# krzkro4122/vit-gan

Hardware: AMD Instinct MI355X
Metric: images/sec (G+D step) ViTGAN 32x32 patch4 dim384 (higher is better)
Workload: dtype bf16; 1 GPU; C2: CIFAR-10-shaped 3x32x32, patch 4 (65 tokens), E=384, 4 heads, 6 blocks ViT discriminator + SLN/SIREN generator (z=1024, 32 tokens, 4 blocks), full alternating G+D step, AdamW; fp8_attention=False, per_gpu_batch=256, global_batch=256, loss=ns, parallelism=dp1, hip_graph=True, compress_mapping_grad=False, fused_real_fake_pass=True, losses_finite=True

## Files before the change

vit-gan_amd/csrc/attention.hip:

```cpp
#include "vg_attn.h"
#include "vg_kernels.h"

typedef long fp8x8;
__device__ __forceinline__ fp8x8 to_fp8(float a0, float a1, float a2, float a3, float a4, float a5, float a6, float a7) {
  int lo = 0, hi = 0;
  lo = __builtin_amdgcn_cvt_pk_fp8_f32(a0, a1, lo, false);
  lo = __builtin_amdgcn_cvt_pk_fp8_f32(a2, a3, lo, true);
  hi = __builtin_amdgcn_cvt_pk_fp8_f32(a4, a5, hi, false);
  hi = __builtin_amdgcn_cvt_pk_fp8_f32(a6, a7, hi, true);
  return (fp8x8)(((unsigned long)(unsigned)hi << 32) | (unsigned long)(unsigned)lo);
}
__device__ __forceinline__ fp8x8 to_fp8(bf16x8 v) {
  return to_fp8(vg_bf2f(v[0]), vg_bf2f(v[1]), vg_bf2f(v[2]), vg_bf2f(v[3]), vg_bf2f(v[4]), vg_bf2f(v[5]), vg_bf2f(v[6]), vg_bf2f(v[7]));
}
__device__ __forceinline__ fp8x8 pack_pair_fp8(f32x4 a, f32x4 b, float mul) {
  return to_fp8(a[0] * mul, a[1] * mul, a[2] * mul, a[3] * mul, b[0] * mul, b[1] * mul, b[2] * mul, b[3] * mul);
}
__device__ __forceinline__ f32x4 vg_mfma_fp8(fp8x8 a, fp8x8 b, f32x4 c) { return __builtin_amdgcn_mfma_f32_16x16x32_fp8_fp8(a, b, c, 0, 0, 0); }
template <bool FP8>
__device__ __forceinline__ f32x4 score_mfma(bf16x8 a, bf16x8 b, f32x4 c) {
  if constexpr (FP8) return vg_mfma_fp8(to_fp8(a), to_fp8(b), c);
  else return vg_mfma(a, b, c);
}
#define VG_P_FP8_SCALE 256.0f

template <int HE>
__device__ __forceinline__ void row_sqnorms(const unsigned char* img, float* out, int rows, int tid, int nthreads) {
  for (int r = tid; r < rows; r += nthreads) {
    float a = 0.f;
#pragma unroll
    for (int c = 0; c < HE / 8; ++c) {
      const bf16x8 v = *(const bf16x8*)(img + lds_off<HE>(r, 8 * c));
#pragma unroll
      for (int j = 0; j < 8; ++j) { const float f = vg_bf2f(v[j]); a += f * f; }
    }
    out[r] = a;
  }
}
__device__ __forceinline__ float l2_dist(float qk, float qn, float kn) { return sqrtf(fmaxf(qn + kn - 2.f * qk, 0.f)); }

template <int HE, int NT, bool L2, bool FP8>
__global__ __launch_bounds__(64 * NT) void vg_attn_fwd_kernel(const bf16* __restrict__ qkv, bf16* __restrict__ o,
                                                              float* __restrict__ lse, int B, int S, int H, float scale,
                                                              const void* __restrict__ zeros) {
  constexpr int KS = HE / 32, DT = HE / 16, KP = (NT + 1) / 2, RP = KP * 32, RK = 16 * NT;
  __shared__ __attribute__((aligned(16))) unsigned char sm[(RK + RP) * HE * 2 + (L2 ? RK * 4 : 0)];
  unsigned char* kl = sm;
  unsigned char* vl = sm + RK * HE * 2;
  float* kn = (float*)(sm + (RK + RP) * HE * 2);
  int b, h;
  if (!attn_block(B, H, b, h)) return;
  const int tid = threadIdx.x, lane = tid & 63, qt = tid >> 6;
  const int g = lane >> 4, li = lane & 15;
  const int E = H * HE;
  const size_t ld = 3 * (size_t)E;
  const bf16* qb = qkv + (size_t)b * S * ld + h * HE;
  const bf16* kb = qb + E;
  const bf16* vb = qb + 2 * E;

  bf16x8 qf[KS];
#pragma unroll
  for (int ks = 0; ks < KS; ++ks) qf[ks] = gfrag(qb, ld, 16 * qt, ks, S, lane);
  dma_head<HE, NT>(kl, kb, ld, S, RK, zeros, qt, lane);
  dma_head<HE, NT>(vl, vb, ld, S, RP, zeros, (qt + 2) % NT, lane);
  asm volatile("s_waitcnt vmcnt(0)" ::: "memory");
  __syncthreads();
  float qn = 0.f;
  if (L2) {
    row_sqnorms<HE>(kl, kn, RK, tid, 64 * NT);
#pragma unroll
    for (int ks = 0; ks < KS; ++ks)
#pragma unroll
      for (int j = 0; j < 8; ++j) { const float f = vg_bf2f(qf[ks][j]); qn += f * f; }
    qn = group_sum(qn);
    __syncthreads();
  }

  f32x4 sc[NT];
#pragma unroll
  for (int kt = 0; kt < NT; ++kt) {
    f32x4 a = {0.f, 0.f, 0.f, 0.f};
#pragma unroll
    for (int ks = 0; ks < KS; ++ks) a = score_mfma<FP8>(lfrag_row<HE>(kl, 16 * kt, ks, lane), qf[ks], a);
    sc[kt] = a;
  }
  const int q = 16 * qt + li;
  float m = -INFINITY;
#pragma unroll
  for (int kt = 0; kt < NT; ++kt)
#pragma unroll
    for (int r = 0; r < 4; ++r) {
      const int key = 16 * kt + 4 * g + r;
      const float raw = L2 ? l2_dist(sc[kt][r], qn, kn[key]) : sc[kt][r];
      const float sv = (key < S) ? raw * scale : -INFINITY;
      sc[kt][r] = sv;
      m = fmaxf(m, sv);
    }
  m = group_max(m);
  float l = 0.f;
#pragma unroll
  for (int kt = 0; kt < NT; ++kt)
#pragma unroll
    for (int r = 0; r < 4; ++r) {
      const float p = __expf(sc[kt][r] - m);
      sc[kt][r] = p;
      l += p;
    }
  l = group_sum(l);
  const float inv_l = 1.0f / l;
  if (g == 0 && q < S) lse[((size_t)b * H + h) * S + q] = m + __logf(l);

  f32x4 oa[DT];
#pragma unroll
  for (int dt = 0; dt < DT; ++dt) oa[dt] = (f32x4){0.f, 0.f, 0.f, 0.f};
#pragma unroll
  for (int u = 0; u < KP; ++u) {
    const f32x4 zero = {0.f, 0.f, 0.f, 0.f};
    const f32x4 hi = (2 * u + 1 < NT) ? sc[(2 * u + 1 < NT) ? 2 * u + 1 : 0] : zero;
    if constexpr (FP8) {
      const fp8x8 pf = pack_pair_fp8(sc[2 * u], hi, VG_P_FP8_SCALE);
#pragma unroll
      for (int dt = 0; dt < DT; ++dt) oa[dt] = vg_mfma_fp8(to_fp8(lfrag_tr<HE>(vl, u, 16 * dt, lane)), pf, oa[dt]);
    } else {
      const bf16x8 pf = pack_pair(sc[2 * u], hi);
#pragma unroll
      for (int dt = 0; dt < DT; ++dt) oa[dt] = vg_mfma(lfrag_tr<HE>(vl, u, 16 * dt, lane), pf, oa[dt]);
    }
  }
  store_tiles<DT>(o + ((size_t)b * S + (q < S ? q : 0)) * E + h * HE, oa, FP8 ? inv_l * (1.0f / VG_P_FP8_SCALE) : inv_l, g, q < S);
}

template <int HE, int NT, bool L2, bool FP8>
__global__ __launch_bounds__(64 * NT, 2) void vg_attn_bwd_kernel(const bf16* __restrict__ qkv, const bf16* __restrict__ o,
                                                         const bf16* __restrict__ d_o, const float* __restrict__ lse,
                                                         bf16* __restrict__ dqkv, int B, int S, int H, float scale,
                                                         const void* __restrict__ zeros) {
  constexpr int KS = HE / 32, DT = HE / 16, KP = (NT + 1) / 2, RP = KP * 32;
  constexpr int IMG = RP * HE * 2;
  __shared__ __attribute__((aligned(16))) unsigned char sm[4 * IMG + (L2 ? 4 : 2) * RP * 4];
  unsigned char* lk = sm;
  unsigned char* lv = sm + IMG;
  unsigned char* lq = sm + 2 * IMG;
  unsigned char* ldo = sm + 3 * IMG;
  float* dl = (float*)(sm + 4 * IMG);
  float* ll = dl + RP;
  float* qn_l = ll + RP;
  float* kn_l = qn_l + RP;
  int b, h;
  if (!attn_block(B, H, b, h)) return;
  const int tid = threadIdx.x, lane = tid & 63, wv = tid >> 6;
  const int g = lane >> 4, li = lane & 15;
  const int E = H * HE;
  const size_t ld = 3 * (size_t)E;
  const bf16* qb = qkv + (size_t)b * S * ld + h * HE;
  const bf16* kb = qb + E;
  const bf16* vb = qb + 2 * E;
  const bf16* ob = o + (size_t)b * S * E + h * HE;
  const bf16* dob = d_o + (size_t)b * S * E + h * HE;
  const float* lb = lse + ((size_t)b * H + h) * S;
  bf16* dqb = dqkv + (size_t)b * S * ld + h * HE;
  const f32x4 zero = {0.f, 0.f, 0.f, 0.f};

  bf16x8 of[KS];
#pragma unroll
  for (int ks = 0; ks < KS; ++ks) of[ks] = gfrag(ob, (size_t)E, 16 * wv, ks, S, lane);
  dma_head<HE, NT>(lk, kb, ld, S, RP, zeros, wv, lane);
  dma_head<HE, NT>(lv, vb, ld, S, RP, zeros, (wv + 1) % NT, lane);
  dma_head<HE, NT>(lq, qb, ld, S, RP, zeros, (wv + 2) % NT, lane);
  dma_head<HE, NT>(ldo, dob, (size_t)E, S, RP, zeros, (wv + 3) % NT, lane);
  for (int i = tid; i < RP; i += 64 * NT) ll[i] = (i < S) ? lb[i] : 0.f;
  asm volatile("s_waitcnt vmcnt(0)" ::: "memory");
  __syncthreads();

  bf16x8 qf[KS], dof[KS];
  {
    float dpart = 0.f;
#pragma unroll
    for (int ks = 0; ks < KS; ++ks) {
      qf[ks] = lfrag_row<HE>(lq, 16 * wv, ks, lane);
      dof[ks] = lfrag_row<HE>(ldo, 16 * wv, ks, lane);
#pragma unroll
      for (int j = 0; j < 8; ++j) dpart += vg_bf2f(dof[ks][j]) * vg_bf2f(of[ks][j]);
    }
    const float delta = group_sum(dpart);
    if (g == 0) dl[16 * wv + li] = delta;
  }
  if (L2) { row_sqnorms<HE>(lq, qn_l, RP, tid, 64 * NT); row_sqnorms<HE>(lk, kn_l, RP, tid, 64 * NT); }
  __syncthreads();

  {
    const int qt = wv;
    const int q = 16 * qt + li;
    const float delta = dl[q];
    const float lse_q = ll[q];
    const float qn = L2 ? qn_l[q] : 0.f;
    float wsum = 0.f;
    f32x4 ds[NT];
#pragma unroll
    for (int kt = 0; kt < NT; ++kt) {
      f32x4 st = zero, dpt = zero;
#pragma unroll
      for (int ks = 0; ks < KS; ++ks) {
        st = score_mfma<FP8>(lfrag_row<HE>(lk, 16 * kt, ks, lane), qf[ks], st);
        dpt = vg_mfma(lfrag_row<HE>(lv, 16 * kt, ks, lane), dof[ks], dpt);
      }
      f32x4 kn4 = zero;
      if (L2) kn4 = *(const f32x4*)(kn_l + 16 * kt + 4 * g);
#pragma unroll
      for (int r = 0; r < 4; ++r) {
        const int key = 16 * kt + 4 * g + r;
        const float raw = L2 ? l2_dist(st[r], qn, kn4[r]) : st[r];
        const float p = (key < S && q < S) ? __expf(raw * scale - lse_q) : 0.f;
        float dsv = p * (dpt[r] - delta) * scale;
        if (L2) { dsv = raw > 0.f ? dsv / raw : 0.f; wsum += dsv; }
        ds[kt][r] = dsv;
      }
    }
    if (L2) wsum = group_sum(wsum);
    f32x4 dq[DT];
#pragma unroll
    for (int dt = 0; dt < DT; ++dt) dq[dt] = zero;
#pragma unroll
    for (int u = 0; u < KP; ++u) {
      const bf16x8 dsf = pack_pair(ds[2 * u], (2 * u + 1 < NT) ? ds[(2 * u + 1 < NT) ? 2 * u + 1 : 0] : zero);
#pragma unroll
      for (int dt = 0; dt < DT; ++dt) dq[dt] = vg_mfma(lfrag_tr<HE>(lk, u, 16 * dt, lane), dsf, dq[dt]);
    }
    if (L2) {
#pragma unroll
      for (int dt = 0; dt < DT; ++dt) {
        const bf16x4 qv = *(const bf16x4*)(lq + lds_off<HE>(q, 16 * dt + 4 * g));
#pragma unroll
        for (int r = 0; r < 4; ++r) dq[dt][r] = wsum * vg_bf2f(qv[r]) - dq[dt][r];
      }
    }
    store_tiles<DT>(dqb + (size_t)(q < S ? q : 0) * ld, dq, 1.0f, g, q < S);
  }
  {
    const int kt = wv;
    const int key = 16 * kt + li;
    bf16x8 kf[KS], vf[KS];
#pragma unroll
    for (int ks = 0; ks < KS; ++ks) {
      kf[ks] = lfrag_row<HE>(lk, 16 * kt, ks, lane);
      vf[ks] = lfrag_row<HE>(lv, 16 * kt, ks, lane);
    }
    f32x4 pr[NT], ds[NT];
    const float kn = L2 ? kn_l[key] : 0.f;
    float wsum = 0.f;
#pragma unroll
    for (int qt = 0; qt < NT; ++qt) {
      f32x4 s = zero, dp = zero;
#pragma unroll
      for (int ks = 0; ks < KS; ++ks) {
        s = score_mfma<FP8>(lfrag_row<HE>(lq, 16 * qt, ks, lane), kf[ks], s);
        dp = vg_mfma(lfrag_row<HE>(ldo, 16 * qt, ks, lane), vf[ks], dp);
      }
      const f32x4 lq4 = *(const f32x4*)(ll + 16 * qt + 4 * g);
      const f32x4 dl4 = *(const f32x4*)(dl + 16 * qt + 4 * g);
      f32x4 qn4 = zero;
      if (L2) qn4 = *(const f32x4*)(qn_l + 16 * qt + 4 * g);
#pragma unroll
      for (int r = 0; r < 4; ++r) {
        const int q = 16 * qt + 4 * g + r;
        const bool ok = (q < S) && (key < S);
        const float raw = L2 ? l2_dist(s[r], qn4[r], kn) : s[r];
        const float p = ok ? __expf(raw * scale - lq4[r]) : 0.f;
        pr[qt][r] = p;
        float dsv = p * (dp[r] - dl4[r]) * scale;
        if (L2) { dsv = raw > 0.f ? dsv / raw : 0.f; wsum += dsv; }
        ds[qt][r] = dsv;
      }
    }
    if (L2) wsum = group_sum(wsum);
    f32x4 dv[DT], dk[DT];
#pragma unroll
    for (int dt = 0; dt < DT; ++dt) { dv[dt] = zero; dk[dt] = zero; }
#pragma unroll
    for (int u = 0; u < KP; ++u) {
      const int hi = (2 * u + 1 < NT) ? 2 * u + 1 : 0;
      const bf16x8 pf = pack_pair(pr[2 * u], (2 * u + 1 < NT) ? pr[hi] : zero);
      const bf16x8 dsf = pack_pair(ds[2 * u], (2 * u + 1 < NT) ? ds[hi] : zero);
#pragma unroll
      for (int dt = 0; dt < DT; ++dt) {
        dv[dt] = vg_mfma(lfrag_tr<HE>(ldo, u, 16 * dt, lane), pf, dv[dt]);
        dk[dt] = vg_mfma(lfrag_tr<HE>(lq, u, 16 * dt, lane), dsf, dk[dt]);
      }
    }
    if (L2) {
#pragma unroll
      for (int dt = 0; dt < DT; ++dt) {
        const bf16x4 kv = *(const bf16x4*)(lk + lds_off<HE>(key, 16 * dt + 4 * g));
#pragma unroll
        for (int r = 0; r < 4; ++r) dk[dt][r] = wsum * vg_bf2f(kv[r]) - dk[dt][r];
      }
    }
    bf16* rowp = dqb + (size_t)(key < S ? key : 0) * ld;
    store_tiles<DT>(rowp + E, dk, 1.0f, g, key < S);
    store_tiles<DT>(rowp + 2 * E, dv, 1.0f, g, key < S);
  }
}

#ifndef VG_ATTN_BWD2_WPE
#define VG_ATTN_BWD2_WPE 5
#endif
template <int HE, int NT, bool FP8>
__global__ __launch_bounds__(64 * NT, VG_ATTN_BWD2_WPE) void vg_attn_bwd2_kernel(const bf16* __restrict__ qkv, const bf16* __restrict__ o,
                                                                  const bf16* __restrict__ d_o, const float* __restrict__ lse,
                                                                  bf16* __restrict__ dqkv, int B, int S, int H, float scale,
                                                                  const void* __restrict__ zeros) {
  constexpr int KS = HE / 32, DT = HE / 16, KP = (NT + 1) / 2, RP = KP * 32;
  constexpr int IMG = RP * HE * 2;
  __shared__ __attribute__((aligned(16))) unsigned char sm[2 * IMG + 2 * RP * 4];
  unsigned char* s0 = sm;
  unsigned char* s1 = sm + IMG;
  float* dl = (float*)(sm + 2 * IMG);
  float* ll = dl + RP;
  int b, h;
  if (!attn_block(B, H, b, h)) return;
  const int tid = threadIdx.x, lane = tid & 63, wv = tid >> 6;
  const int g = lane >> 4, li = lane & 15;
  const int E = H * HE;
  const size_t ld = 3 * (size_t)E;
  const bf16* qb = qkv + (size_t)b * S * ld + h * HE;
  const bf16* kb = qb + E;
  const bf16* vb = qb + 2 * E;
  const bf16* ob = o + (size_t)b * S * E + h * HE;
  const bf16* dob = d_o + (size_t)b * S * E + h * HE;
  const float* lb = lse + ((size_t)b * H + h) * S;
  bf16* dqb = dqkv + (size_t)b * S * ld + h * HE;
  const f32x4 zero = {0.f, 0.f, 0.f, 0.f};

  dma_head<HE, NT>(s0, kb, ld, S, RP, zeros, wv, lane);
  dma_head<HE, NT>(s1, vb, ld, S, RP, zeros, (wv + 1) % NT, lane);
  bf16x8 qf[KS], dof[KS];
  {
    bf16x8 of[KS];
#pragma unroll
    for (int ks = 0; ks < KS; ++ks) {
      of[ks] = gfrag(ob, (size_t)E, 16 * wv, ks, S, lane);
      dof[ks] = gfrag(dob, (size_t)E, 16 * wv, ks, S, lane);
      qf[ks] = gfrag(qb, ld, 16 * wv, ks, S, lane);
    }
    for (int i = tid; i < RP; i += 64 * NT) ll[i] = (i < S) ? lb[i] : 0.f;
    float dpart = 0.f;
#pragma unroll
    for (int ks = 0; ks < KS; ++ks) {
#pragma unroll
      for (int j = 0; j < 8; ++j) dpart += vg_bf2f(dof[ks][j]) * vg_bf2f(of[ks][j]);
    }
    const float delta = group_sum(dpart);
    if (g == 0) dl[16 * wv + li] = delta;
  }
  asm volatile("s_waitcnt vmcnt(0)" ::: "memory");
  __syncthreads();

  {
    const int q = 16 * wv + li;
    const float delta = dl[q];
    const float lse_q = ll[q];
    f32x4 ds[NT];
#pragma unroll
    for (int kt = 0; kt < NT; ++kt) {
      f32x4 st = zero, dpt = zero;
#pragma unroll
      for (int ks = 0; ks < KS; ++ks) {
        st = score_mfma<FP8>(lfrag_row<HE>(s0, 16 * kt, ks, lane), qf[ks], st);
        dpt = vg_mfma(lfrag_row<HE>(s1, 16 * kt, ks, lane), dof[ks], dpt);
      }
#pragma unroll
      for (int r = 0; r < 4; ++r) {
        const int key = 16 * kt + 4 * g + r;
        const float p = (key < S && q < S) ? __expf(st[r] * scale - lse_q) : 0.f;
        ds[kt][r] = p * (dpt[r] - delta) * scale;
      }
    }
    bf16x8 dsf[KP];
#pragma unroll
    for (int u = 0; u < KP; ++u) dsf[u] = pack_pair(ds[2 * u], (2 * u + 1 < NT) ? ds[(2 * u + 1 < NT) ? 2 * u + 1 : 0] : zero);
    bf16* rowq = dqb + (size_t)(q < S ? q : 0) * ld;
#pragma unroll
    for (int pp = 0; pp < DT / 2; ++pp) {
      f32x4 dq[2] = {zero, zero};
#pragma unroll
      for (int u = 0; u < KP; ++u) {
        dq[0] = vg_mfma(lfrag_tr<HE>(s0, u, 32 * pp, lane), dsf[u], dq[0]);
        dq[1] = vg_mfma(lfrag_tr<HE>(s0, u, 32 * pp + 16, lane), dsf[u], dq[1]);
      }
      store_tiles<2>(rowq + 32 * pp, dq, 1.0f, g, q < S);
    }
  }
  bf16x8 kf[KS], vf[KS];
#pragma unroll
  for (int ks = 0; ks < KS; ++ks) {
    kf[ks] = lfrag_row<HE>(s0, 16 * wv, ks, lane);
    vf[ks] = lfrag_row<HE>(s1, 16 * wv, ks, lane);
  }
  __syncthreads();
  dma_head<HE, NT>(s0, qb, ld, S, RP, zeros, wv, lane);
  dma_head<HE, NT>(s1, dob, (size_t)E, S, RP, zeros, (wv + 1) % NT, lane);
  asm volatile("s_waitcnt vmcnt(0)" ::: "memory");
  __syncthreads();
  {
    const int key = 16 * wv + li;
    f32x4 pr[NT], ds[NT];
#pragma unroll
    for (int qt = 0; qt < NT; ++qt) {
      f32x4 s = zero, dp = zero;
#pragma unroll
      for (int ks = 0; ks < KS; ++ks) {
        s = score_mfma<FP8>(lfrag_row<HE>(s0, 16 * qt, ks, lane), kf[ks], s);
        dp = vg_mfma(lfrag_row<HE>(s1, 16 * qt, ks, lane), vf[ks], dp);
      }
      const f32x4 lq4 = *(const f32x4*)(ll + 16 * qt + 4 * g);
      const f32x4 dl4 = *(const f32x4*)(dl + 16 * qt + 4 * g);
#pragma unroll
      for (int r = 0; r < 4; ++r) {
        const int q = 16 * qt + 4 * g + r;
        const float p = ((q < S) && (key < S)) ? __expf(s[r] * scale - lq4[r]) : 0.f;
        pr[qt][r] = p;
        ds[qt][r] = p * (dp[r] - dl4[r]) * scale;
      }
    }
    bf16x8 pf[KP], dsf[KP];
#pragma unroll
    for (int u = 0; u < KP; ++u) {
      const int hi = (2 * u + 1 < NT) ? 2 * u + 1 : 0;
      pf[u] = pack_pair(pr[2 * u], (2 * u + 1 < NT) ? pr[hi] : zero);
      dsf[u] = pack_pair(ds[2 * u], (2 * u + 1 < NT) ? ds[hi] : zero);
    }
    bf16* rowp = dqb + (size_t)(key < S ? key : 0) * ld;
#pragma unroll
    for (int pp = 0; pp < DT / 2; ++pp) {
      f32x4 dv[2] = {zero, zero}, dk[2] = {zero, zero};
#pragma unroll
      for (int u = 0; u < KP; ++u) {
#pragma unroll
        for (int t = 0; t < 2; ++t) {
          dv[t] = vg_mfma(lfrag_tr<HE>(s1, u, 32 * pp + 16 * t, lane), pf[u], dv[t]);
          dk[t] = vg_mfma(lfrag_tr<HE>(s0, u, 32 * pp + 16 * t, lane), dsf[u], dk[t]);
        }
      }
      store_tiles<2>(rowp + E + 32 * pp, dk, 1.0f, g, key < S);
      store_tiles<2>(rowp + 2 * E + 32 * pp, dv, 1.0f, g, key < S);
    }
  }
}

template <int HE>
__global__ __launch_bounds__(320, 2) void vg_attn_bwd_bwd2_kernel(const bf16* __restrict__ qkv, const bf16* __restrict__ d_o,
                                                                  const float* __restrict__ lse, const bf16* __restrict__ uqkv,
                                                                  bf16* __restrict__ d_do, bf16* __restrict__ d_qkv, int B, int S, int H,
                                                                  float scale, const void* __restrict__ zeros) {
  constexpr int NT = 5, KS = HE / 32, DT = HE / 16, KP = 3, RP = 96;
  constexpr int IMG = RP * HE * 2;
  __shared__ __attribute__((aligned(16))) unsigned char sm[4 * IMG + 4 * RP * 4];
  unsigned char* i0 = sm;
  unsigned char* i1 = sm + IMG;
  unsigned char* i2 = sm + 2 * IMG;
  unsigned char* i3 = sm + 3 * IMG;
  float* dl = (float*)(sm + 4 * IMG);
  float* gm = dl + RP;
  float* pl = gm + RP;
  float* ll = pl + RP;
  int b, h;
  if (!attn_block(B, H, b, h)) return;
  const int tid = threadIdx.x, lane = tid & 63, wv = tid >> 6;
  const int g = lane >> 4, li = lane & 15;
  const int E = H * HE;
  const size_t ld = 3 * (size_t)E;
  const bf16* qb = qkv + (size_t)b * S * ld + h * HE;
  const bf16* kb = qb + E;
  const bf16* vb = qb + 2 * E;
  const bf16* uqb = uqkv + (size_t)b * S * ld + h * HE;
  const bf16* ukb = uqb + E;
  const bf16* uvb = uqb + 2 * E;
  const bf16* dob = d_o + (size_t)b * S * E + h * HE;
  const float* lb = lse + ((size_t)b * H + h) * S;
  bf16* ddob = d_do + (size_t)b * S * E + h * HE;
  bf16* dqb = d_qkv + (size_t)b * S * ld + h * HE;
  const f32x4 zero = {0.f, 0.f, 0.f, 0.f};

  dma_head<HE, NT>(i0, kb, ld, S, RP, zeros, wv, lane);
  dma_head<HE, NT>(i1, vb, ld, S, RP, zeros, (wv + 1) % NT, lane);
  dma_head<HE, NT>(i2, ukb, ld, S, RP, zeros, (wv + 2) % NT, lane);
  dma_head<HE, NT>(i3, uvb, ld, S, RP, zeros, (wv + 3) % NT, lane);
  bf16x8 qf[KS], dof[KS], uqf[KS];
#pragma unroll
  for (int ks = 0; ks < KS; ++ks) {
    qf[ks] = gfrag(qb, ld, 16 * wv, ks, S, lane);
    dof[ks] = gfrag(dob, (size_t)E, 16 * wv, ks, S, lane);
    uqf[ks] = gfrag(uqb, ld, 16 * wv, ks, S, lane);
  }
  for (int i = tid; i < RP; i += 64 * NT) ll[i] = (i < S) ? lb[i] : 0.f;
  asm volatile("s_waitcnt vmcnt(0)" ::: "memory");
  __syncthreads();

  {
    const int q = 16 * wv + li;
    const float lse_q = ll[q];
    f32x4 Pm[NT], Dm[NT], Gm[NT], Tm[NT];
    float delta = 0.f, gam = 0.f;
#pragma unroll
    for (int kt = 0; kt < NT; ++kt) {
      f32x4 st = zero, dpt = zero, gt = zero, tt = zero;
#pragma unroll
      for (int ks = 0; ks < KS; ++ks) {
        const bf16x8 kr = lfrag_row<HE>(i0, 16 * kt, ks, lane);
        st = vg_mfma(kr, qf[ks], st);
        gt = vg_mfma(kr, uqf[ks], gt);
        gt = vg_mfma(lfrag_row<HE>(i2, 16 * kt, ks, lane), qf[ks], gt);
        dpt = vg_mfma(lfrag_row<HE>(i1, 16 * kt, ks, lane), dof[ks], dpt);
        tt = vg_mfma(lfrag_row<HE>(i3, 16 * kt, ks, lane), dof[ks], tt);
      }
#pragma unroll
      for (int r = 0; r < 4; ++r) {
        const int key = 16 * kt + 4 * g + r;
        const float p = (key < S && q < S) ? __expf(st[r] * scale - lse_q) : 0.f;
        const float gv = gt[r] * scale;
        Pm[kt][r] = p; Dm[kt][r] = dpt[r]; Gm[kt][r] = gv; Tm[kt][r] = tt[r];
        delta += p * dpt[r];
        gam += p * gv;
      }
    }
    delta = group_sum(delta);
    gam = group_sum(gam);
    float pis = 0.f;
#pragma unroll
    for (int kt = 0; kt < NT; ++kt)
#pragma unroll
      for (int r = 0; r < 4; ++r) {
        const float a = Dm[kt][r] - delta;
        const float pie = Tm[kt][r] + Gm[kt][r] * a - gam * Dm[kt][r];
        Tm[kt][r] = pie;
        Dm[kt][r] = a;
        pis += Pm[kt][r] * pie;
      }
    pis = group_sum(pis);
    if (g == 0) { dl[q] = delta; gm[q] = gam; pl[q] = pis; }
#pragma unroll
    for (int kt = 0; kt < NT; ++kt)
#pragma unroll
      for (int r = 0; r < 4; ++r) {
        const float p = Pm[kt][r];
        Gm[kt][r] = p * (Gm[kt][r] - gam);
        Dm[kt][r] = p * Dm[kt][r];
        Tm[kt][r] = p * (Tm[kt][r] - pis);
      }
    bf16x8 pf[KP], hf[KP], dsf[KP], sgf[KP];
#pragma unroll
    for (int u = 0; u < KP; ++u) {
      const bool two = 2 * u + 1 < NT;
      const int hi = two ? 2 * u + 1 : 0;
      pf[u] = pack_pair(Pm[2 * u], two ? Pm[hi] : zero);
      hf[u] = pack_pair(Gm[2 * u], two ? Gm[hi] : zero);
      dsf[u] = pack_pair(Dm[2 * u], two ? Dm[hi] : zero);
      sgf[u] = pack_pair(Tm[2 * u], two ? Tm[hi] : zero);
    }
    bf16* rowo = ddob + (size_t)(q < S ? q : 0) * E;
    bf16* rowq = dqb + (size_t)(q < S ? q : 0) * ld;
#pragma unroll
    for (int pp = 0; pp < DT / 2; ++pp) {
      f32x4 o1[2] = {zero, zero}, o2[2] = {zero, zero};
#pragma unroll
      for (int u = 0; u < KP; ++u)
#pragma unroll
        for (int t = 0; t < 2; ++t) {
          const int d0 = 32 * pp + 16 * t;
          o1[t] = vg_mfma(lfrag_tr<HE>(i3, u, d0, lane), pf[u], o1[t]);
          o1[t] = vg_mfma(lfrag_tr<HE>(i1, u, d0, lane), hf[u], o1[t]);
          o2[t] = vg_mfma(lfrag_tr<HE>(i2, u, d0, lane), dsf[u], o2[t]);
          o2[t] = vg_mfma(lfrag_tr<HE>(i0, u, d0, lane), sgf[u], o2[t]);
        }
      store_tiles<2>(rowo + 32 * pp, o1, 1.0f, g, q < S);
      store_tiles<2>(rowq + 32 * pp, o2, scale, g, q < S);
    }
  }
  bf16x8 kf[KS], vf[KS], ukf[KS], uvf[KS];
#pragma unroll
  for (int ks = 0; ks < KS; ++ks) {
    kf[ks] = lfrag_row<HE>(i0, 16 * wv, ks, lane);
    vf[ks] = lfrag_row<HE>(i1, 16 * wv, ks, lane);
    ukf[ks] = lfrag_row<HE>(i2, 16 * wv, ks, lane);
    uvf[ks] = lfrag_row<HE>(i3, 16 * wv, ks, lane);
  }
  __syncthreads();
  dma_head<HE, NT>(i0, qb, ld, S, RP, zeros, wv, lane);
  dma_head<HE, NT>(i1, dob, (size_t)E, S, RP, zeros, (wv + 1) % NT, lane);
  dma_head<HE, NT>(i2, uqb, ld, S, RP, zeros, (wv + 2) % NT, lane);
  asm volatile("s_waitcnt vmcnt(0)" ::: "memory");
  __syncthreads();
  {
    const int key = 16 * wv + li;
    f32x4 Hm[NT], Dm[NT], Sm[NT];
#pragma unroll
    for (int qt = 0; qt < NT; ++qt) {
      f32x4 st = zero, dpt = zero, gt = zero, tt = zero;
#pragma unroll
      for (int ks = 0; ks < KS; ++ks) {
        const bf16x8 qr = lfrag_row<HE>(i0, 16 * qt, ks, lane);
        const bf16x8 dr = lfrag_row<HE>(i1, 16 * qt, ks, lane);
        st = vg_mfma(qr, kf[ks], st);
        gt = vg_mfma(qr, ukf[ks], gt);
        gt = vg_mfma(lfrag_row<HE>(i2, 16 * qt, ks, lane), kf[ks], gt);
        dpt = vg_mfma(dr, vf[ks], dpt);
        tt = vg_mfma(dr, uvf[ks], tt);
      }
      const f32x4 lq4 = *(const f32x4*)(ll + 16 * qt + 4 * g);
      const f32x4 dl4 = *(const f32x4*)(dl + 16 * qt + 4 * g);
      const f32x4 gm4 = *(const f32x4*)(gm + 16 * qt + 4 * g);
      const f32x4 pl4 = *(const f32x4*)(pl + 16 * qt + 4 * g);
#pragma unroll
      for (int r = 0; r < 4; ++r) {
        const int q = 16 * qt + 4 * g + r;
        const float p = ((q < S) && (key < S)) ? __expf(st[r] * scale - lq4[r]) : 0.f;
        const float gv = gt[r] * scale, a = dpt[r] - dl4[r];
        const float pie = tt[r] + gv * a - gm4[r] * dpt[r];
        Hm[qt][r] = p * (gv - gm4[r]);
        Dm[qt][r] = p * a;
        Sm[qt][r] = p * (pie - pl4[r]);
      }
    }
    bf16x8 hf[KP], dsf[KP], sgf[KP];
#pragma unroll
    for (int u = 0; u < KP; ++u) {
      const bool two = 2 * u + 1 < NT;
      const int hi = two ? 2 * u + 1 : 0;
      hf[u] = pack_pair(Hm[2 * u], two ? Hm[hi] : zero);
      dsf[u] = pack_pair(Dm[2 * u], two ? Dm[hi] : zero);
      sgf[u] = pack_pair(Sm[2 * u], two ? Sm[hi] : zero);
    }
    bf16* rowp = dqb + (size_t)(key < S ? key : 0) * ld;
#pragma unroll
    for (int pp = 0; pp < DT / 2; ++pp) {
      f32x4 dk[2] = {zero, zero}, dv[2] = {zero, zero};
#pragma unroll
      for (int u = 0; u < KP; ++u)
#pragma unroll
        for (int t = 0; t < 2; ++t) {
          const int d0 = 32 * pp + 16 * t;
          dk[t] = vg_mfma(lfrag_tr<HE>(i2, u, d0, lane), dsf[u], dk[t]);
          dk[t] = vg_mfma(lfrag_tr<HE>(i0, u, d0, lane), sgf[u], dk[t]);
          dv[t] = vg_mfma(lfrag_tr<HE>(i1, u, d0, lane), hf[u], dv[t]);
        }
      store_tiles<2>(rowp + E + 32 * pp, dk, scale, g, key < S);
      store_tiles<2>(rowp + 2 * E + 32 * pp, dv, 1.0f, g, key < S);
    }
  }
}

__device__ __attribute__((aligned(16))) unsigned int vg_attn_zero_page[4] = {0u, 0u, 0u, 0u};
static const void* attn_zeros() {
  static void* zp = nullptr;
  if (!zp && hipGetSymbolAddress(&zp, HIP_SYMBOL(vg_attn_zero_page)) != hipSuccess) zp = nullptr;
  return zp;
}

template <int HE, int NT, int MODE>
static int launch_fwd(const bf16* qkv, bf16* o, float* lse, int B, int H, int S, float scale, hipStream_t st) {
  const void* z = attn_zeros();
  if (!z) return -5;
  hipLaunchKernelGGL((vg_attn_fwd_kernel<HE, NT, MODE == 1, MODE == 2>), dim3(attn_grid(B, H)), dim3(64 * NT), 0, st, qkv, o, lse, B, S, H, scale, z);
  return (int)hipGetLastError();
}
template <int HE, int NT, int MODE>
static int launch_bwd(const bf16* qkv, const bf16* o, const bf16* d_o, const float* lse, bf16* dqkv, int B, int H,
                      int S, float scale, hipStream_t st) {
  const void* z = attn_zeros();
  if (!z) return -5;
#ifndef VG_ATTN_BWD_4IMG
  if constexpr (MODE != 1 && NT == 5) {
    hipLaunchKernelGGL((vg_attn_bwd2_kernel<HE, NT, MODE == 2>), dim3(attn_grid(B, H)), dim3(64 * NT), 0, st, qkv, o, d_o, lse, dqkv, B, S, H, scale, z);
    return (int)hipGetLastError();
  }
#endif
  hipLaunchKernelGGL((vg_attn_bwd_kernel<HE, NT, MODE == 1, MODE == 2>), dim3(attn_grid(B, H)), dim3(64 * NT), 0, st, qkv, o, d_o, lse, dqkv, B, S, H, scale, z);
  return (int)hipGetLastError();
}

#define VG_ATTN_BY_NT(FN, HE_, MODE_, ...) return small ? FN<HE_, 2, MODE_>(__VA_ARGS__) : FN<HE_, 5, MODE_>(__VA_ARGS__)
#define VG_ATTN_BY_MODE(FN, HE_, ...)                                  \
  do {                                                                 \
    if (mode == 0) { VG_ATTN_BY_NT(FN, HE_, 0, __VA_ARGS__); }         \
    if (mode == 1) { VG_ATTN_BY_NT(FN, HE_, 1, __VA_ARGS__); }         \
    VG_ATTN_BY_NT(FN, HE_, 2, __VA_ARGS__);                            \
  } while (0)
#define VG_ATTN_DISPATCH(FN, ...)                                      \
  do {                                                                 \
    if (S < 1 || S > 80 || B < 1 || H < 1) return -2;                  \
    if (mode < 0 || mode > 2) return -4;                               \
    const bool small = (S <= 32);                                      \
    if (HE == 96) VG_ATTN_BY_MODE(FN, 96, __VA_ARGS__);                \
    if (HE == 64) VG_ATTN_BY_MODE(FN, 64, __VA_ARGS__);                \
    if (HE == 32) VG_ATTN_BY_MODE(FN, 32, __VA_ARGS__);                \
    return -3;                                                         \
  } while (0)
int vg_attn_fwd_launch(const bf16* qkv, bf16* o, float* lse, int B, int H, int S, int HE, float scale, int mode, hipStream_t st) {
  if (mode == 0 && S > VG_SHORT_MAX_S && S <= VG_ATTN_LONG_MAX_S) return vg_attn_long_fwd_launch(qkv, o, lse, B, H, S, HE, scale, st);
  VG_ATTN_DISPATCH(launch_fwd, qkv, o, lse, B, H, S, scale, st);
}
int vg_attn_bwd_launch(const bf16* qkv, const bf16* o, const bf16* d_o, const float* lse, bf16* dqkv, int B, int H,
                       int S, int HE, float scale, int mode, hipStream_t st) {
  if (mode == 0 && S > VG_SHORT_MAX_S && S <= VG_ATTN_LONG_MAX_S) return vg_attn_long_bwd_launch(qkv, o, d_o, lse, dqkv, B, H, S, HE, scale, st);
  VG_ATTN_DISPATCH(launch_bwd, qkv, o, d_o, lse, dqkv, B, H, S, scale, st);
}

template <int HE, int KMAX>
__global__ __launch_bounds__(64) void vg_attn_cls_fwd_kernel(const bf16* __restrict__ qkv, bf16* __restrict__ o_cls, float* __restrict__ lse_cls,
                                                             int B, int S, int H, float scale) {
  constexpr int CPR = HE / 8, RPI = 64 / CPR;
  __shared__ float q0l[HE];
  constexpr int NR = KMAX / 64;
  __shared__ float part[KMAX * CPR];
  __shared__ float pl[KMAX];
  int b, h;
  if (!attn_block(B, H, b, h)) return;
  const int lane = threadIdx.x;
  const int rr = lane / CPR, c = lane - rr * CPR;
  const bool act = rr < RPI;
  const int E = H * HE;
  const size_t ld = 3 * (size_t)E;
  const bf16* qb = qkv + (size_t)b * S * ld + h * HE;
  const bf16* kb = qb + E;
  const bf16* vb = qb + 2 * E;
  for (int d = lane; d < HE; d += 64) q0l[d] = vg_bf2f(qb[d]);
  __syncthreads();
  float qc[8];
#pragma unroll
  for (int t = 0; t < 8; ++t) qc[t] = q0l[8 * (act ? c : 0) + t];
  for (int r0 = 0; r0 < S; r0 += RPI) {
    const int r = r0 + rr;
    if (act && r < S) {
      const bf16x8 k8 = *(const bf16x8*)(kb + (size_t)r * ld + 8 * c);
      float a = 0.f;
#pragma unroll
      for (int t = 0; t < 8; ++t) a = fmaf(qc[t], vg_bf2f(k8[t]), a);
      part[r * CPR + c] = a;
    }
  }
  __syncthreads();
  float sv[NR];
#pragma unroll
  for (int rnd = 0; rnd < NR; ++rnd) {
    const int j = lane + 64 * rnd;
    float a = 0.f;
    if (j < S) {
#pragma unroll
      for (int cc = 0; cc < CPR; ++cc) a += part[j * CPR + cc];
    }
    sv[rnd] = (j < S) ? a * scale : -INFINITY;
  }
  float mx = sv[0];
#pragma unroll
  for (int rnd = 1; rnd < NR; ++rnd) mx = fmaxf(mx, sv[rnd]);
  const float m = vg_wave_max(mx);
  float pv[NR], ps = 0.f;
#pragma unroll
  for (int rnd = 0; rnd < NR; ++rnd) { pv[rnd] = __expf(sv[rnd] - m); ps = rnd ? ps + pv[rnd] : pv[rnd]; }
  const float l = vg_wave_sum(ps);
#pragma unroll
  for (int rnd = 0; rnd < NR; ++rnd) pl[lane + 64 * rnd] = vg_bf2f(vg_f2bf(pv[rnd]));
  if (lane == 0) lse_cls[(size_t)b * H + h] = m + __logf(l);
  __syncthreads();
  float oa[8];
#pragma unroll
  for (int t = 0; t < 8; ++t) oa[t] = 0.f;
  for (int r0 = 0; r0 < S; r0 += RPI) {
    const int r = r0 + rr;
    if (act && r < S) {
      const bf16x8 v8 = *(const bf16x8*)(vb + (size_t)r * ld + 8 * c);
      const float pj = pl[r];
#pragma unroll
      for (int t = 0; t < 8; ++t) oa[t] = fmaf(pj, vg_bf2f(v8[t]), oa[t]);
    }
  }
#pragma unroll
  for (int t = 0; t < 8; ++t) part[lane * 8 + t] = oa[t];
  __syncthreads();
  const float inv_l = 1.0f / l;
  for (int d = lane; d < HE; d += 64) {
    float a = 0.f;
#pragma unroll
    for (int q = 0; q < RPI; ++q) a += part[(q * CPR + (d >> 3)) * 8 + (d & 7)];
    o_cls[(size_t)b * E + h * HE + d] = vg_f2bf(a * inv_l);
  }
}

template <int HE, int KMAX>
__global__ __launch_bounds__(64) void vg_attn_cls_bwd_kernel(const bf16* __restrict__ qkv, const bf16* __restrict__ o_cls, const bf16* __restrict__ do_cls,
                                                             const float* __restrict__ lse_cls, bf16* __restrict__ dqkv, int B, int S, int H,
                                                             float scale) {
  constexpr int CPR = HE / 8, RPI = 64 / CPR;
  __shared__ float q0l[HE], d0l[HE];
  __shared__ float ps[KMAX * CPR], pd[KMAX * CPR];
  __shared__ float dsl[KMAX], pbl[KMAX];
  int b, h;
  if (!attn_block(B, H, b, h)) return;
  const int lane = threadIdx.x;
  const int rr = lane / CPR, c = lane - rr * CPR;
  const bool act = rr < RPI;
  const int E = H * HE;
  const size_t ld = 3 * (size_t)E;
  const bf16* qb = qkv + (size_t)b * S * ld + h * HE;
  const bf16* kb = qb + E;
  const bf16* vb = qb + 2 * E;
  bf16* dqb = dqkv + (size_t)b * S * ld + h * HE;
  const float lse0 = lse_cls[(size_t)b * H + h];
  float dpart = 0.f;
  for (int d = lane; d < HE; d += 64) {
    q0l[d] = vg_bf2f(qb[d]);
    const float dv = vg_bf2f(do_cls[(size_t)b * E + h * HE + d]);
    d0l[d] = dv;
    dpart = fmaf(dv, vg_bf2f(o_cls[(size_t)b * E + h * HE + d]), dpart);
  }
  const float delta = vg_wave_sum(dpart);
  __syncthreads();
  float qc[8], dc[8];
#pragma unroll
  for (int t = 0; t < 8; ++t) { qc[t] = q0l[8 * (act ? c : 0) + t]; dc[t] = d0l[8 * (act ? c : 0) + t]; }
  for (int r0 = 0; r0 < S; r0 += RPI) {
    const int r = r0 + rr;
    if (act && r < S) {
      const bf16x8 k8 = *(const bf16x8*)(kb + (size_t)r * ld + 8 * c);
      const bf16x8 v8 = *(const bf16x8*)(vb + (size_t)r * ld + 8 * c);
      float a = 0.f, e = 0.f;
#pragma unroll
      for (int t = 0; t < 8; ++t) { a = fmaf(qc[t], vg_bf2f(k8[t]), a); e = fmaf(dc[t], vg_bf2f(v8[t]), e); }
      ps[r * CPR + c] = a;
      pd[r * CPR + c] = e;
    }
  }
  __syncthreads();
#pragma unroll
  for (int rnd = 0; rnd < KMAX / 64; ++rnd) {
    const int j = lane + 64 * rnd;
    float dsv = 0.f, pb = 0.f;
    if (j < S) {
      float sc = 0.f, dp = 0.f;
#pragma unroll
      for (int cc = 0; cc < CPR; ++cc) { sc += ps[j * CPR + cc]; dp += pd[j * CPR + cc]; }
      const float p = __expf(sc * scale - lse0);
      dsv = vg_bf2f(vg_f2bf(p * (dp - delta) * scale));
      pb = vg_bf2f(vg_f2bf(p));
    }
    dsl[j] = dsv;
    pbl[j] = pb;
  }
  __syncthreads();
  float qa[8];
#pragma unroll
  for (int t = 0; t < 8; ++t) qa[t] = 0.f;
  for (int r0 = 0; r0 < S; r0 += RPI) {
    const int r = r0 + rr;
    if (act && r < S) {
      const bf16x8 k8 = *(const bf16x8*)(kb + (size_t)r * ld + 8 * c);
      const float dj = dsl[r], pj = pbl[r];
      bf16x8 dk8, dv8;
#pragma unroll
      for (int t = 0; t < 8; ++t) {
        dk8[t] = vg_f2bf(dj * qc[t]);
        dv8[t] = vg_f2bf(pj * dc[t]);
        qa[t] = fmaf(dj, vg_bf2f(k8[t]), qa[t]);
      }
      bf16* rowp = dqb + (size_t)r * ld + 8 * c;
      *(bf16x8*)(rowp + E) = dk8;
      *(bf16x8*)(rowp + 2 * E) = dv8;
      if (r > 0) *(u32x4*)rowp = (u32x4){0u, 0u, 0u, 0u};
    }
  }
#pragma unroll
  for (int t = 0; t < 8; ++t) ps[lane * 8 + t] = qa[t];
  __syncthreads();
  for (int d = lane; d < HE; d += 64) {
    float a = 0.f;
#pragma unroll
    for (int q = 0; q < RPI; ++q) a += ps[(q * CPR + (d >> 3)) * 8 + (d & 7)];
    dqb[d] = vg_f2bf(a);
  }
}

int vg_attn_cls_fwd_launch(const bf16* qkv, bf16* o_cls, float* lse_cls, int B, int H, int S, int HE, float scale, hipStream_t st) {
  if (S < 1 || S > VG_ATTN_LONG_MAX_S || B < 1 || H < 1) return -2;
#define VG_ACLS(HE_, K_) hipLaunchKernelGGL((vg_attn_cls_fwd_kernel<HE_, K_>), dim3(attn_grid(B, H)), dim3(64), 0, st, qkv, o_cls, lse_cls, B, S, H, scale)
#define VG_ACLS_K(K_) if (HE == 96) VG_ACLS(96, K_); else if (HE == 64) VG_ACLS(64, K_); else if (HE == 32) VG_ACLS(32, K_); else return -3
  if (S <= 128) { VG_ACLS_K(128); } else { VG_ACLS_K(256); }
#undef VG_ACLS_K
#undef VG_ACLS
  return (int)hipGetLastError();
}
int vg_attn_cls_bwd_launch(const bf16* qkv, const bf16* o_cls, const bf16* do_cls, const float* lse_cls, bf16* dqkv, int B, int H, int S, int HE,
                           float scale, hipStream_t st) {
  if (S < 1 || S > VG_ATTN_LONG_MAX_S || B < 1 || H < 1) return -2;
#define VG_ACLS(HE_, K_) hipLaunchKernelGGL((vg_attn_cls_bwd_kernel<HE_, K_>), dim3(attn_grid(B, H)), dim3(64), 0, st, qkv, o_cls, do_cls, lse_cls, dqkv, B, S, H, scale)
#define VG_ACLS_K(K_) if (HE == 96) VG_ACLS(96, K_); else if (HE == 64) VG_ACLS(64, K_); else if (HE == 32) VG_ACLS(32, K_); else return -3
  if (S <= 128) { VG_ACLS_K(128); } else { VG_ACLS_K(256); }
#undef VG_ACLS_K
#undef VG_ACLS
  return (int)hipGetLastError();
}

int vg_attn_bwd_bwd_mfma_launch(const bf16* qkv, const bf16* d_o, const float* lse, const bf16* uqkv, bf16* d_do, bf16* d_qkv, int B, int H,
                                int S, int HE, float scale, hipStream_t st) {
  if (S < 1 || S > 80 || B < 1 || H < 1) return -2;
  const void* z = attn_zeros();
  if (!z) return -5;
#define VG_ABB2(HE_) hipLaunchKernelGGL((vg_attn_bwd_bwd2_kernel<HE_>), dim3(attn_grid(B, H)), dim3(320), 0, st, qkv, d_o, lse, uqkv, d_do, d_qkv, B, S, H, scale, z)
  if (HE == 96) VG_ABB2(96); else if (HE == 64) VG_ABB2(64); else if (HE == 32) VG_ABB2(32); else return -3;
#undef VG_ABB2
  return (int)hipGetLastError();
}
```

Before: 48870 images/sec.

## Compute P and dS once in attention backward, reuse dS tile for dQ

Adds a new attention-backward kernel that computes the score and dP matrices only once, in the key-major pass, instead of recomputing them in a separate query-major pass for dQ. dS is written to a bank-swizzled LDS tile and read back transposed with ds_read_tr16 to feed the dQ MFMAs, removing one full set of S and dP MFMAs plus the exp work. The default dispatch now uses this kernel, and the old one sits behind a macro. It also adds compile-gated s_memtime stamps for profiling, and it costs an extra LDS tile, a write and transpose-read round trip, and an extra barrier.

```diff
diff --git a/vit-gan_amd/csrc/attention.hip b/vit-gan_amd/csrc/attention.hip
--- a/vit-gan_amd/csrc/attention.hip
+++ b/vit-gan_amd/csrc/attention.hip
@@ -301,6 +301,13 @@
   }
 }
 
+#if defined(VG_TUNING) && defined(VG_ATTN_STAMPS)
+#define VG_ATTN_NSTAMP 8
+__device__ unsigned long long vg_attn_stamp_buf[8192 * VG_ATTN_NSTAMP];
+#define VG_ASTAMP(i) do { if (threadIdx.x == 0 && blockIdx.x < 8192) vg_attn_stamp_buf[blockIdx.x * VG_ATTN_NSTAMP + (i)] = __builtin_amdgcn_s_memtime(); } while (0)
+#else
+#define VG_ASTAMP(i) do { } while (0)
+#endif
 #ifndef VG_ATTN_BWD2_WPE
 #define VG_ATTN_BWD2_WPE 5
 #endif
@@ -330,6 +337,7 @@
   const float* lb = lse + ((size_t)b * H + h) * S;
   bf16* dqb = dqkv + (size_t)b * S * ld + h * HE;
   const f32x4 zero = {0.f, 0.f, 0.f, 0.f};
+  VG_ASTAMP(0);
 
   dma_head<HE, NT>(s0, kb, ld, S, RP, zeros, wv, lane);
   dma_head<HE, NT>(s1, vb, ld, S, RP, zeros, (wv + 1) % NT, lane);
@@ -354,6 +362,7 @@
   }
   asm volatile("s_waitcnt vmcnt(0)" ::: "memory");
   __syncthreads();
+  VG_ASTAMP(1);
 
   {
     const int q = 16 * wv + li;
@@ -378,6 +387,7 @@
     bf16x8 dsf[KP];
 #pragma unroll
     for (int u = 0; u < KP; ++u) dsf[u] = pack_pair(ds[2 * u], (2 * u + 1 < NT) ? ds[(2 * u + 1 < NT) ? 2 * u + 1 : 0] : zero);
+    VG_ASTAMP(2);
     bf16* rowq = dqb + (size_t)(q < S ? q : 0) * ld;
 #pragma unroll
     for (int pp = 0; pp < DT / 2; ++pp) {
@@ -390,6 +400,7 @@
       store_tiles<2>(rowq + 32 * pp, dq, 1.0f, g, q < S);
     }
   }
+  VG_ASTAMP(3);
   bf16x8 kf[KS], vf[KS];
 #pragma unroll
   for (int ks = 0; ks < KS; ++ks) {
@@ -401,6 +412,7 @@
   dma_head<HE, NT>(s1, dob, (size_t)E, S, RP, zeros, (wv + 1) % NT, lane);
   asm volatile("s_waitcnt vmcnt(0)" ::: "memory");
   __syncthreads();
+  VG_ASTAMP(4);
   {
     const int key = 16 * wv + li;
     f32x4 pr[NT], ds[NT];
@@ -429,6 +441,7 @@
       pf[u] = pack_pair(pr[2 * u], (2 * u + 1 < NT) ? pr[hi] : zero);
       dsf[u] = pack_pair(ds[2 * u], (2 * u + 1 < NT) ? ds[hi] : zero);
     }
+    VG_ASTAMP(5);
     bf16* rowp = dqb + (size_t)(key < S ? key : 0) * ld;
 #pragma unroll
     for (int pp = 0; pp < DT / 2; ++pp) {
@@ -445,6 +458,156 @@
       store_tiles<2>(rowp + 2 * E + 32 * pp, dv, 1.0f, g, key < S);
     }
   }
+  VG_ASTAMP(6);
+}
+
+#ifndef VG_ATTN_BWD1_WPE
+#define VG_ATTN_BWD1_WPE 5
+#endif
+__device__ __forceinline__ int ds_tile_off(int key, int q) {
+  const int c = q * 2 + (((key >> 3) & 1) << 4);
+  return key * 160 + (c >= 160 ? c - 160 : c);
+}
+template <int HE, int NT, bool FP8>
+__global__ __launch_bounds__(64 * NT, VG_ATTN_BWD1_WPE) void vg_attn_bwd1_kernel(const bf16* __restrict__ qkv, const bf16* __restrict__ o,
+                                                                  const bf16* __restrict__ d_o, const float* __restrict__ lse,
+                                                                  bf16* __restrict__ dqkv, int B, int S, int H, float scale,
+                                                                  const void* __restrict__ zeros) {
+  static_assert(NT == 5, "the dS tile's pitch and bank map are those of 80 queries");
+  constexpr int KS = HE / 32, DT = HE / 16, KP = (NT + 1) / 2, RP = KP * 32;
+  constexpr int IMG = RP * HE * 2;
+  constexpr int TSZ = 16 * NT * 160, I0 = IMG > TSZ ? IMG : TSZ;
+  __shared__ __attribute__((aligned(16))) unsigned char sm[I0 + IMG + 2 * RP * 4];
+  unsigned char* s0 = sm;
+  unsigned char* s1 = sm + I0;
+  float* dl = (float*)(sm + I0 + IMG);
+  float* ll = dl + RP;
+  unsigned char* ts = s0;
+  int b, h;
+  if (!attn_block(B, H, b, h)) return;
+  VG_ASTAMP(0);
+  const int tid = threadIdx.x, lane = tid & 63, wv = tid >> 6;
+  const int g = lane >> 4, li = lane & 15;
+  const int E = H * HE;
+  const size_t ld = 3 * (size_t)E;
+  const bf16* qb = qkv + (size_t)b * S * ld + h * HE;
+  const bf16* kb = qb + E;
+  const bf16* vb = qb + 2 * E;
+  const bf16* ob = o + (size_t)b * S * E + h * HE;
+  const bf16* dob = d_o + (size_t)b * S * E + h * HE;
+  const float* lb = lse + ((size_t)b * H + h) * S;
+  bf16* dqb = dqkv + (size_t)b * S * ld + h * HE;
+  const f32x4 zero = {0.f, 0.f, 0.f, 0.f};
+
+  dma_head<HE, NT>(s0, qb, ld, S, RP, zeros, wv, lane);
+  dma_head<HE, NT>(s1, dob, (size_t)E, S, RP, zeros, (wv + 1) % NT, lane);
+  bf16x8 kf[KS], vf[KS];
+  {
+    bf16x8 of[KS], dof[KS];
+#pragma unroll
+    for (int ks = 0; ks < KS; ++ks) {
+      of[ks] = gfrag(ob, (size_t)E, 16 * wv, ks, S, lane);
+      dof[ks] = gfrag(dob, (size_t)E, 16 * wv, ks, S, lane);
+      kf[ks] = gfrag(kb, ld, 16 * wv, ks, S, lane);
+      vf[ks] = gfrag(vb, ld, 16 * wv, ks, S, lane);
+    }
+    for (int i = tid; i < RP; i += 64 * NT) ll[i] = (i < S) ? lb[i] : 0.f;
+    float dpart = 0.f;
+#pragma unroll
+    for (int ks = 0; ks < KS; ++ks) {
+#pragma unroll
+      for (int j = 0; j < 8; ++j) dpart += vg_bf2f(dof[ks][j]) * vg_bf2f(of[ks][j]);
+    }
+    const float delta = group_sum(dpart);
+    if (g == 0) dl[16 * wv + li] = delta;
+  }
+  asm volatile("s_waitcnt vmcnt(0)" ::: "memory");
+  __syncthreads();
+  VG_ASTAMP(1);
+
+  const int key = 16 * wv + li;
+  bf16x8 pf[KP], dsf[KP];
+  {
+    f32x4 pr[NT], ds[NT];
+#pragma unroll
+    for (int qt = 0; qt < NT; ++qt) {
+      f32x4 s = zero, dp = zero;
+#pragma unroll
+      for (int ks = 0; ks < KS; ++ks) {
+        s = score_mfma<FP8>(lfrag_row<HE>(s0, 16 * qt, ks, lane), kf[ks], s);
+        dp = vg_mfma(lfrag_row<HE>(s1, 16 * qt, ks, lane), vf[ks], dp);
+      }
+      const f32x4 lq4 = *(const f32x4*)(ll + 16 * qt + 4 * g);
+      const f32x4 dl4 = *(const f32x4*)(dl + 16 * qt + 4 * g);
+#pragma unroll
+      for (int r = 0; r < 4; ++r) {
+        const int q = 16 * qt + 4 * g + r;
+        const float p = ((q < S) && (key < S)) ? __expf(s[r] * scale - lq4[r]) : 0.f;
+        pr[qt][r] = p;
+        ds[qt][r] = p * (dp[r] - dl4[r]) * scale;
+      }
+    }
+#pragma unroll
+    for (int u = 0; u < KP; ++u) {
+      const int hi = (2 * u + 1 < NT) ? 2 * u + 1 : 0;
+      pf[u] = pack_pair(pr[2 * u], (2 * u + 1 < NT) ? pr[hi] : zero);
+      dsf[u] = pack_pair(ds[2 * u], (2 * u + 1 < NT) ? ds[hi] : zero);
+    }
+  }
+  VG_ASTAMP(2);
+  bf16* rowp = dqb + (size_t)(key < S ? key : 0) * ld;
+#pragma unroll
+  for (int pp = 0; pp < DT / 2; ++pp) {
+    f32x4 dv[2] = {zero, zero}, dk[2] = {zero, zero};
+#pragma unroll
+    for (int u = 0; u < KP; ++u) {
+#pragma unroll
+      for (int t = 0; t < 2; ++t) {
+        dv[t] = vg_mfma(lfrag_tr<HE>(s1, u, 32 * pp + 16 * t, lane), pf[u], dv[t]);
+        dk[t] = vg_mfma(lfrag_tr<HE>(s0, u, 32 * pp + 16 * t, lane), dsf[u], dk[t]);
+      }
+    }
+    store_tiles<2>(rowp + E + 32 * pp, dk, 1.0f, g, key < S);
+    store_tiles<2>(rowp + 2 * E + 32 * pp, dv, 1.0f, g, key < S);
+  }
+  __syncthreads();
+  dma_head<HE, NT>(s1, kb, ld, S, RP, zeros, wv, lane);
+#pragma unroll
+  for (int qt = 0; qt < NT; ++qt) {
+    bf16x4 w;
+#pragma unroll
+    for (int r = 0; r < 4; ++r) w[r] = dsf[qt >> 1][4 * (qt & 1) + r];
+    *(bf16x4*)(ts + ds_tile_off(key, 16 * qt + 4 * g)) = w;
+  }
+  VG_ASTAMP(3);
+  asm volatile("s_waitcnt vmcnt(0)" ::: "memory");
+  __syncthreads();
+  {
+    const int q = 16 * wv + li;
+    typedef bf16x4 __attribute__((address_space(3))) * lds4;
+    bf16x8 dsq[KP];
+#pragma unroll
+    for (int u = 0; u < KP; ++u) {
+      const int kr = 32 * u + 4 * g + (li >> 2), qc = 16 * wv + 4 * (li & 3);
+      const bf16x4 lo = __builtin_amdgcn_ds_read_tr16_b64_v4bf16((lds4)(ts + ds_tile_off(kr, qc)));
+      bf16x4 hi = {0, 0, 0, 0};
+      if (2 * u + 1 < NT) hi = __builtin_amdgcn_ds_read_tr16_b64_v4bf16((lds4)(ts + ds_tile_off(kr + 16, qc)));
+      dsq[u][0] = lo[0]; dsq[u][1] = lo[1]; dsq[u][2] = lo[2]; dsq[u][3] = lo[3];
+      dsq[u][4] = hi[0]; dsq[u][5] = hi[1]; dsq[u][6] = hi[2]; dsq[u][7] = hi[3];
+    }
+    bf16* rowq = dqb + (size_t)(q < S ? q : 0) * ld;
+#pragma unroll
+    for (int pp = 0; pp < DT / 2; ++pp) {
+      f32x4 dq[2] = {zero, zero};
+#pragma unroll
+      for (int u = 0; u < KP; ++u) {
+        dq[0] = vg_mfma(lfrag_tr<HE>(s1, u, 32 * pp, lane), dsq[u], dq[0]);
+        dq[1] = vg_mfma(lfrag_tr<HE>(s1, u, 32 * pp + 16, lane), dsq[u], dq[1]);
+      }
+      store_tiles<2>(rowq + 32 * pp, dq, 1.0f, g, q < S);
+    }
+  }
+  VG_ASTAMP(4);
 }
 
 template <int HE>
@@ -670,7 +833,11 @@
   if (!z) return -5;
 #ifndef VG_ATTN_BWD_4IMG
   if constexpr (MODE != 1 && NT == 5) {
+#ifdef VG_ATTN_BWD_2IMG
     hipLaunchKernelGGL((vg_attn_bwd2_kernel<HE, NT, MODE == 2>), dim3(attn_grid(B, H)), dim3(64 * NT), 0, st, qkv, o, d_o, lse, dqkv, B, S, H, scale, z);
+#else
+    hipLaunchKernelGGL((vg_attn_bwd1_kernel<HE, NT, MODE == 2>), dim3(attn_grid(B, H)), dim3(64 * NT), 0, st, qkv, o, d_o, lse, dqkv, B, S, H, scale, z);
+#endif
     return (int)hipGetLastError();
   }
 #endif
@@ -909,3 +1076,9 @@
 #undef VG_ABB2
   return (int)hipGetLastError();
 }
+
+#if defined(VG_TUNING) && defined(VG_ATTN_STAMPS)
+extern "C" int vg_attn_debug_stamps(unsigned long long* host, int n) {
+  return (int)hipMemcpyFromSymbol(host, HIP_SYMBOL(vg_attn_stamp_buf), (size_t)n * sizeof(unsigned long long), 0, hipMemcpyDeviceToHost);
+}
+#endif
```

After: 49040 images/sec, median of 6. About the same (+0.3%).
